# twice154/ofa-for-super-resolution

Measured on AMD Instinct MI355X. Metric: sr_training_images_per_sec_4x_64to256, higher is better.
Workload: dtype bf16; 1 GPU; OFA-SR S4 supernet 4x progressive shrinking (elastic kernel {3,5,7}, e=6, d=4, pd=2), LR 64x64 -> HR 256x256, fwd+bwd+Adam, train-mode BN; kernel_transform_mode=1, compat_reference_indexing=True, parallelism=dp1, per_gpu_batch=16, global_batch=16, grad_allreduce_bytes=0, launch=eager

## Files before the change

### ofa-for-super-resolution_amd/csrc/conv2d.hip

```cpp
#include "ofasr_common.h"

namespace ofasr {

typedef __attribute__((ext_vector_type(16))) float cv_f32x16;
typedef __attribute__((ext_vector_type(8))) __bf16 cv_bf16x8;
typedef __attribute__((ext_vector_type(8))) _Float16 cv_f16x8;
typedef __attribute__((ext_vector_type(8))) short cv_s16x8;

constexpr int CV_TW = 64;
constexpr int CV_SEG = 20;
constexpr int CV_RP = 4 * CV_SEG;
constexpr int CV_KC = 32;

template <typename T> struct CvMma;
template <> struct CvMma<bf16_t> {
    static __device__ __forceinline__ cv_f32x16 run(cv_s16x8 a, cv_s16x8 b, cv_f32x16 c) {
        return __builtin_amdgcn_mfma_f32_32x32x16_bf16(__builtin_bit_cast(cv_bf16x8, a), __builtin_bit_cast(cv_bf16x8, b),
                                                       c, 0, 0, 0);
    }
};
template <> struct CvMma<f16_t> {
    static __device__ __forceinline__ cv_f32x16 run(cv_s16x8 a, cv_s16x8 b, cv_f32x16 c) {
        return __builtin_amdgcn_mfma_f32_32x32x16_f16(__builtin_bit_cast(cv_f16x8, a), __builtin_bit_cast(cv_f16x8, b), c,
                                                      0, 0, 0);
    }
};

__device__ __forceinline__ int cv_pos(int r, int col) { return r * CV_RP + (col & 3) * CV_SEG + (col >> 2); }
__device__ __forceinline__ int cv_rec(int P, int j) { return P * 64 + ((j ^ ((P >> 2) & 3)) << 4); }

struct CvBn {
    float* ss;
    const float* gamma;
    const float* beta;
    const float* mean;
    const float* var;
    float eps;
};

template <typename T>
__global__ void __launch_bounds__(256) conv_prep_kernel(const float* __restrict__ w, T* __restrict__ wimg, int Cin,
                                                        int KS, int dgrad, int M, int Kdim, int nrb, long long total,
                                                        CvBn bn) {
    const long long idx = (long long)blockIdx.x * blockDim.x + threadIdx.x;
    if (bn.ss != nullptr && idx < M) {
        float sc = 1.f, sh = 0.f;
        if (bn.gamma != nullptr) {
            sc = bn.gamma[idx] * rsqrtf(bn.var[idx] + bn.eps);
            sh = bn.beta[idx] - bn.mean[idx] * sc;
        }
        bn.ss[idx] = sc;
        bn.ss[M + idx] = sh;
    }
    if (idx >= total) return;
    const int j = (int)(idx & 7), lane = (int)((idx >> 3) & 63);
    long long t = idx >> 9;
    const int rb = (int)(t % nrb);
    t /= nrb;
    const int tx = (int)(t % KS);
    t /= KS;
    const int s = (int)(t & 1);
    t >>= 1;
    const int ty = (int)(t % KS);
    const int kc = (int)(t / KS);
    const int m = rb * 32 + (lane & 31), kk = kc * CV_KC + 16 * s + 8 * (lane >> 5) + j;
    float v = 0.f;
    if (m < M && kk < Kdim) {
        const int taps = KS * KS, tap = ty * KS + tx;
        v = dgrad ? w[((long long)kk * Cin + m) * taps + (taps - 1 - tap)]
                  : w[((long long)m * Cin + kk) * taps + tap];
    }
    wimg[idx] = from_float<T>(v);
}

__device__ __forceinline__ void cv_lds_barrier() { asm volatile("s_waitcnt lgkmcnt(0)\n\ts_barrier" ::: "memory"); }

struct CvEpi {
    const float* ss;
    int act;
    float2* stat;
    int P;
};

template <typename T, int KS, int RB, int WM, int WP, bool ONEK>
__global__ void __launch_bounds__(64 * WM * WP, 2) conv_igemm_kernel(const T* __restrict__ x, const T* __restrict__ wimg,
                                                                     T* __restrict__ y, int Cx, int M, int H, int W,
                                                                     int tiles_x, int nkc, int nrb, CvEpi epi) {
    constexpr int THREADS = 64 * WM * WP;
    constexpr int PAD = KS / 2;
    constexpr int TH = 2 * WP;
    constexpr int RH = TH + KS - 1;
    constexpr int RW = CV_TW + KS - 1;
    constexpr int NIT = 2 * KS;
    __shared__ __attribute__((aligned(16))) char Xt[RH * CV_RP * 64];

    const int tile = blockIdx.x;
    const int ty0 = (tile / tiles_x) * TH, tx0 = (tile % tiles_x) * CV_TW;
    const int n = blockIdx.y, slab = blockIdx.z;
    const int tid = threadIdx.x;
    const int lane = lane_id();
    const int wave = __builtin_amdgcn_readfirstlane((int)(threadIdx.x >> 6));
    const int wm = wave % WM, wp = wave / WM;
    const int c = lane & 31, h = lane >> 5;
    const int prow = 2 * wp + (c >> 4), pcol = 4 * (c & 15);
    const int grb0 = (slab * WM + wm) * RB;

    const int P0 = prow * CV_RP + (c & 15);
    int bbase[2][4][2];
#pragma unroll
    for (int cs = 0; cs < 2; ++cs)
#pragma unroll
        for (int m = 0; m < 4; ++m)
#pragma unroll
            for (int ks = 0; ks < 2; ++ks) {
                const int key = (((P0 >> 2) & 3) + m + (cs && (c & 3) == 3 ? 1 : 0)) & 3;
                bbase[cs][m][ks] = P0 * 64 + (((2 * ks + h) ^ key) << 4);
            }
    auto read_b = [&](int ty, int u, int ks) -> cv_s16x8 {
        const int D = ty * CV_RP + (u & 3) * CV_SEG + (u >> 2);
        return *reinterpret_cast<const cv_s16x8*>(Xt + bbase[u >> 2][(D >> 2) & 3][ks] + D * 64);
    };

    cv_f32x16 acc[RB][4];
#pragma unroll
    for (int rb = 0; rb < RB; ++rb)
#pragma unroll
        for (int t = 0; t < 4; ++t)
#pragma unroll
            for (int i = 0; i < 16; ++i) acc[rb][t][i] = 0.f;

    const T* xn = x + (long long)n * Cx * H * W;
    const uint4* wbase = reinterpret_cast<const uint4*>(wimg);
    for (int kc = 0; kc < nkc; ++kc) {
        cv_s16x8 A[KS][RB];
        const long long it_stride = (long long)KS * nrb * 64;
        const uint4* wk = wbase + (long long)kc * NIT * it_stride + (long long)grb0 * 64;
#pragma unroll
        for (int tx = 0; tx < KS; ++tx)
#pragma unroll
            for (int rb = 0; rb < RB; ++rb)
                A[tx][rb] = __builtin_bit_cast(cv_s16x8, (wk + ((long long)tx * nrb + rb) * 64)[lane]);

        cv_lds_barrier();
        constexpr int NRUN = (CV_TW + 16) / 8;
        constexpr int NTASK = 4 * RH * NRUN;
#pragma unroll 1
        for (int q = tid; q < NTASK; q += THREADS) {
            const int run = q % NRUN;
            const int r = (q / NRUN) % RH;
            const int g = q / (NRUN * RH);
            const int gy = ty0 - PAD + r;
            const int gx = tx0 - 8 + 8 * run;
            const bool inb = gy >= 0 && gy < H && gx >= 0 && gx < W;
            const int cbase = CV_KC * kc + 8 * g;
            uint4 v[8];
#pragma unroll
            for (int i = 0; i < 8; ++i) {
                v[i] = make_uint4(0, 0, 0, 0);
                if (inb && cbase + i < Cx)
                    v[i] = *reinterpret_cast<const uint4*>(xn + ((long long)(cbase + i) * H + gy) * W + gx);
            }
#pragma unroll
            for (int k = 0; k < 4; ++k) {
                uint32_t lo[4], hi[4];
#pragma unroll
                for (int m = 0; m < 4; ++m) {
                    const uint32_t a = k == 0 ? v[2 * m].x : k == 1 ? v[2 * m].y : k == 2 ? v[2 * m].z : v[2 * m].w;
                    const uint32_t b = k == 0 ? v[2 * m + 1].x : k == 1 ? v[2 * m + 1].y : k == 2 ? v[2 * m + 1].z
                                                                                                  : v[2 * m + 1].w;
                    lo[m] = __builtin_amdgcn_perm(b, a, 0x05040100u);
                    hi[m] = __builtin_amdgcn_perm(b, a, 0x07060302u);
                }
                const int tc0 = 8 * run - 8 + PAD + 2 * k;
                if (tc0 >= 0 && tc0 < RW)
                    *reinterpret_cast<uint4*>(Xt + cv_rec(cv_pos(r, tc0), g)) = make_uint4(lo[0], lo[1], lo[2], lo[3]);
                if (tc0 + 1 >= 0 && tc0 + 1 < RW)
                    *reinterpret_cast<uint4*>(Xt + cv_rec(cv_pos(r, tc0 + 1), g)) = make_uint4(hi[0], hi[1], hi[2], hi[3]);
            }
        }
        cv_lds_barrier();

        constexpr int STEP = ONEK ? 2 : 1;
#pragma unroll
        for (int it = 0; it < NIT; it += STEP) {
            const int ty = it >> 1, ks = it & 1;
            cv_s16x8 B[8];
#pragma unroll
            for (int u = 0; u < KS + 3; ++u) B[u] = read_b(ty, u, ks);
#pragma unroll
            for (int tx = 0; tx < KS; ++tx) {
#pragma unroll
                for (int rb = 0; rb < RB; ++rb)
#pragma unroll
                    for (int t = 0; t < 4; ++t) acc[rb][t] = CvMma<T>::run(A[tx][rb], B[t + tx], acc[rb][t]);
                __builtin_amdgcn_sched_barrier(0);
                if (it + STEP < NIT) {
#pragma unroll
                    for (int rb = 0; rb < RB; ++rb)
                        A[tx][rb] = __builtin_bit_cast(
                            cv_s16x8, (wk + (it + STEP) * it_stride + ((long long)tx * nrb + rb) * 64)[lane]);
                }
                __builtin_amdgcn_sched_barrier(0);
            }
        }
    }
    const int oy = ty0 + prow, ox = tx0 + pcol;
    if (epi.ss != nullptr) {
        if (oy >= H || ox >= W) return;
#pragma unroll
        for (int rb = 0; rb < RB; ++rb) {
            const int mb = (grb0 + rb) * 32 + 4 * h;
#pragma unroll
            for (int q = 0; q < 4; ++q) {
                float v[4][4];
#pragma unroll
                for (int j = 0; j < 4; ++j) {
                    const int m = mb + 8 * q + j;
                    const int mc = m < M ? m : M - 1;
                    const float sc = epi.ss[mc], sh = epi.ss[M + mc];
#pragma unroll
                    for (int t = 0; t < 4; ++t) {
                        float r = fmaf(acc[rb][t][4 * q + j], sc, sh);
                        if (epi.act == 1) r = fminf(fmaxf(r, 0.f), 6.f);
                        v[j][t] = r;
                    }
                }
                if (epi.act == 2) {
                    const int m0 = mb + 8 * q;
                    if (m0 < M) {
                        T* dst = y + (((long long)n * (M >> 2) + (m0 >> 2)) * (2 * H) + 2 * oy) * (2 * W) + 2 * ox;
#pragma unroll
                        for (int dy = 0; dy < 2; ++dy)
                            *reinterpret_cast<uint4*>(dst + (long long)dy * (2 * W)) =
                                make_uint4(pack2<T>(v[2 * dy][0], v[2 * dy + 1][0]), pack2<T>(v[2 * dy][1], v[2 * dy + 1][1]),
                                           pack2<T>(v[2 * dy][2], v[2 * dy + 1][2]), pack2<T>(v[2 * dy][3], v[2 * dy + 1][3]));
                    }
                } else {
#pragma unroll
                    for (int j = 0; j < 4; ++j) {
                        const int m = mb + 8 * q + j;
                        if (m < M)
                            *reinterpret_cast<uint2*>(y + (((long long)n * M + m) * H + oy) * W + ox) =
                                make_uint2(pack2<T>(v[j][0], v[j][1]), pack2<T>(v[j][2], v[j][3]));
                    }
                }
            }
        }
        return;
    }
    const bool inside = oy < H && ox < W;
    if (inside) {
#pragma unroll
        for (int rb = 0; rb < RB; ++rb) {
#pragma unroll
            for (int reg = 0; reg < 16; ++reg) {
                const int m = (grb0 + rb) * 32 + (reg & 3) + 8 * (reg >> 2) + 4 * h;
                if (m < M) {
                    T* dst = y + (((long long)n * M + m) * H + oy) * W + ox;
                    *reinterpret_cast<uint2*>(dst) = make_uint2(pack2<T>(acc[rb][0][reg], acc[rb][1][reg]),
                                                                pack2<T>(acc[rb][2][reg], acc[rb][3][reg]));
                }
            }
        }
    }
    if (epi.stat != nullptr) {
        const int unit = (n * (int)gridDim.x + tile) * WP + wp;
#pragma unroll
        for (int rb = 0; rb < RB; ++rb) {
            float sv[16], qv[16];
#pragma unroll
            for (int reg = 0; reg < 16; ++reg) {
                float ss = 0.f, qq = 0.f;
#pragma unroll
                for (int t = 0; t < 4; ++t) {
                    const float v = inside ? to_float(from_float<T>(acc[rb][t][reg])) : 0.f;
                    ss += v;
                    qq = fmaf(v, v, qq);
                }
                sv[reg] = ss;
                qv[reg] = qq;
            }
            half_wave_row_sums(sv, qv, c);
            const int rho = half_wave_row_reg(c);
            const int m = (grb0 + rb) * 32 + (rho & 3) + 8 * (rho >> 2) + 4 * h;
            if ((c & 1) == 0 && m < M) epi.stat[(long long)m * epi.P + unit] = make_float2(sv[0], qv[0]);
        }
    }
}

struct CvPlan {
    bool ok;
    int cfg;
    int rows, th, threads, nslab, nrb, nkc, M, Kdim;
    size_t img_bytes;
};

static CvPlan cv_plan(int64_t Cin, int64_t Cout, int K, int dgrad, int64_t N = 0, int64_t H = 0, int64_t W = 0) {
    CvPlan p{};
    p.M = (int)(dgrad ? Cin : Cout);
    p.Kdim = (int)(dgrad ? Cout : Cin);
    p.ok = (K == 3 || K == 5) && p.M > 0 && p.Kdim > 0;
    p.cfg = p.M > 128 ? 0 : (p.M > 64 ? 1 : (p.M > 32 ? 2 : 3));
    if (p.cfg == 2 && N > 0 && N * cdiv(H, 8) * cdiv(W, CV_TW) < 512) p.cfg = 4;
    p.rows = p.cfg == 0 ? 256 : (p.cfg == 1 ? 128 : (p.cfg == 3 ? 32 : 64));
    p.th = p.cfg == 0 ? 2 : ((p.cfg == 1 || p.cfg == 4) ? 4 : 8);
    p.threads = 256;
    p.nslab = (int)cdiv(p.M, p.rows);
    p.nrb = p.nslab * (p.rows / 32);
    p.nkc = (int)cdiv(p.Kdim, CV_KC);
    p.img_bytes = (size_t)p.nkc * K * 2 * K * p.nrb * 1024;
    return p;
}

template <typename T>
static int launch_conv_prep(const char* name, const float* w, int64_t Cin, int64_t Cout, int K, int dgrad, void* ws, CvBn bn,
                            hipStream_t st) {
    const CvPlan p = cv_plan(Cin, Cout, K, dgrad);
    const long long total = (long long)(p.img_bytes / 2);
    OFASR_LAUNCH((conv_prep_kernel<T>), dim3((unsigned)cdiv(total, 256)), dim3(256), 0, st, w, (T*)ws, (int)Cin, K,
                       dgrad, p.M, p.Kdim, p.nrb, total, bn);
    return check_launch(name);
}

template <typename T>
static int launch_conv_run(const char* name, const void* x, const void* ws, void* y, int64_t N, int64_t Cin, int64_t Cout,
                           int64_t H, int64_t W, int K, int dgrad, CvEpi epi, hipStream_t st) {
    const CvPlan p = cv_plan(Cin, Cout, K, dgrad, N, H, W);
    const int tiles_x = (int)cdiv(W, CV_TW), tiles_y = (int)cdiv(H, p.th);
    dim3 grid((unsigned)(tiles_x * tiles_y), (unsigned)N, (unsigned)p.nslab);
    prof_note((double)sizeof(T) * (double)N * (double)H * (double)W * (double)(Cin + Cout),
              2.0 * (double)N * (double)H * (double)W * (double)Cin * (double)Cout * K * K);
#define OFASR_CV(KS, RB, WM, WP, ONEK)                                                                                  \
    OFASR_LAUNCH((conv_igemm_kernel<T, KS, RB, WM, WP, ONEK>), grid, dim3(64 * WM * WP), 0, st, (const T*)x,         \
                       (const T*)ws, (T*)y, p.Kdim, p.M, (int)H, (int)W, tiles_x, p.nkc, p.nrb, epi)
#define OFASR_CVK(KS, ONEK)                                                                                         \
    switch (p.cfg) {                                                                                                \
        case 0: OFASR_CV(KS, 2, 4, 1, ONEK); break;                                                                 \
        case 1: OFASR_CV(KS, 2, 2, 2, ONEK); break;                                                                 \
        case 2: OFASR_CV(KS, 2, 1, 4, ONEK); break;                                                                 \
        case 4: OFASR_CV(KS, 1, 2, 2, ONEK); break;                                                                 \
        default: OFASR_CV(KS, 1, 1, 4, ONEK); break;                                                                \
    }
    const bool onek = p.Kdim <= 16;
    if (K == 5) {
        if (onek) { OFASR_CVK(5, true) } else { OFASR_CVK(5, false) }
    } else {
        if (onek) { OFASR_CVK(3, true) } else { OFASR_CVK(3, false) }
    }
#undef OFASR_CVK
#undef OFASR_CV
    return check_launch(name);
}

template <typename T>
static int launch_conv2d(const char* name, const void* x, const float* w, void* y, int64_t N, int64_t Cin, int64_t Cout,
                         int64_t H, int64_t W, int K, int dgrad, void* ws, hipStream_t st, StatOut so = StatOut{nullptr, 0}) {
    int rc = launch_conv_prep<T>(name, w, Cin, Cout, K, dgrad, ws, CvBn{}, st);
    if (rc) return rc;
    return launch_conv_run<T>(name, x, ws, y, N, Cin, Cout, H, W, K, dgrad, CvEpi{nullptr, 0, so.partial, so.P}, st);
}

typedef __attribute__((ext_vector_type(4))) short cv_s16x4;
typedef __attribute__((address_space(3))) cv_s16x4 cv_lds_s16x4;

struct CvWgParams {
    int Cin, Cout, H, W, tiles_x, tiles_y, ntiles, ksplit, ncislab, nz;
};

template <int WCI> __device__ __forceinline__ int cvw_xoff(int R, int chunk) {
    if constexpr (WCI == 2) return R * 128 + ((((chunk >> 2) ^ ((R >> 1) & 1))) << 6) + ((chunk & 3) << 4);
    else return R * 64 + (chunk << 4);
}

template <typename T, int KS, int RBW, int WCO, int WCI, int WK>
__global__ void __launch_bounds__(256, 2) conv_wgrad_kernel(const T* __restrict__ dy, const T* __restrict__ x,
                                                            float* __restrict__ part, CvWgParams P) {
    static_assert(WCO * WCI * WK == 4, "4 waves");
    constexpr int PAD = KS / 2;
    constexpr int CIB = 32 * WCI;
    constexpr int REC = 2 * CIB;
    constexpr int ROWS = 32 * RBW * WCO;
    constexpr int XW = 80;
    __shared__ __attribute__((aligned(16))) char Yt[ROWS * 256];
    __shared__ __attribute__((aligned(16))) char Xt[2 * XW * REC];

    const int G = KS * P.nz;
    const int xcd = blockIdx.x & 7, jb = blockIdx.x >> 3;
    const int group = jb % G, split = (jb / G) * 8 + xcd;
    if (split >= P.ksplit) return;
    const int ty = group % KS, z = group / KS;
    const int coslab = z / P.ncislab, cislab = z % P.ncislab;
    const int tid = threadIdx.x, lane = lane_id();
    const int wave = __builtin_amdgcn_readfirstlane((int)(threadIdx.x >> 6));
    const int wco = wave % WCO, wci = (wave / WCO) % WCI, wk = wave / (WCO * WCI);
    const int c = lane & 31, h = lane >> 5;
    const int g = lane >> 4, q = (lane >> 2) & 3, pp = lane & 3;

    int xbase[2][2];
    {
        const int L = 8 * (g >> 1) + q;
        const int cb = 64 * wci + 32 * (g & 1) + 8 * pp;
#pragma unroll
        for (int b1 = 0; b1 < 2; ++b1)
#pragma unroll
            for (int b0 = 0; b0 < 2; ++b0) {
                if constexpr (WCI == 2) {
                    const int bit1 = ((L >> 1) & 1) ^ b1 ^ (b0 & L & 1);
                    xbase[b1][b0] = L * 128 + ((wci ^ bit1) << 6) + (cb & 63);
                } else {
                    xbase[b1][b0] = L * 64 + cb;
                }
            }
    }
    cv_f32x16 acc[RBW][KS];
#pragma unroll
    for (int rb = 0; rb < RBW; ++rb)
#pragma unroll
        for (int tx = 0; tx < KS; ++tx)
#pragma unroll
            for (int i = 0; i < 16; ++i) acc[rb][tx][i] = 0.f;

    const long long HW = (long long)P.H * P.W;
    const int t0 = (int)((long long)split * P.ntiles / P.ksplit), t1 = (int)((long long)(split + 1) * P.ntiles / P.ksplit);
    const int tpi = P.tiles_x * P.tiles_y;
    for (int tile = t0; tile < t1; ++tile) {
        const int n = tile / tpi, trem = tile - n * tpi;
        const int ty0 = (trem / P.tiles_x) * 2, tx0 = (trem % P.tiles_x) * CV_TW;
        const T* xn = x + (long long)n * P.Cin * HW;
        const T* dyn = dy + (long long)n * P.Cout * HW;
        __syncthreads();
        constexpr int NXT = (CIB / 8) * 2 * 10;
        if (tid < NXT) {
            const int run = tid % 10, r = (tid / 10) & 1, cg = tid / 20;
            const int gy = ty0 + r + ty - PAD, gx = tx0 - 8 + 8 * run;
            const bool inb = gy >= 0 && gy < P.H && gx >= 0 && gx < P.W;
            const int cbase = cislab * CIB + 8 * cg;
            uint4 v[8];
            uint32_t okm[8];
#pragma unroll
            for (int i = 0; i < 8; ++i) {
                const bool ok = inb && cbase + i < P.Cin;
                okm[i] = ok ? 0xffffffffu : 0u;
                v[i] = *reinterpret_cast<const uint4*>(xn + (ok ? ((long long)(cbase + i) * P.H + gy) * P.W + gx : 0));
            }
#pragma unroll
            for (int i = 0; i < 8; ++i) {
                v[i].x &= okm[i]; v[i].y &= okm[i]; v[i].z &= okm[i]; v[i].w &= okm[i];
            }
#pragma unroll
            for (int k = 0; k < 4; ++k) {
                uint32_t lo[4], hi[4];
#pragma unroll
                for (int m = 0; m < 4; ++m) {
                    const uint32_t a = k == 0 ? v[2 * m].x : k == 1 ? v[2 * m].y : k == 2 ? v[2 * m].z : v[2 * m].w;
                    const uint32_t b = k == 0 ? v[2 * m + 1].x : k == 1 ? v[2 * m + 1].y : k == 2 ? v[2 * m + 1].z
                                                                                                  : v[2 * m + 1].w;
                    lo[m] = __builtin_amdgcn_perm(b, a, 0x05040100u);
                    hi[m] = __builtin_amdgcn_perm(b, a, 0x07060302u);
                }
                const int R = r * XW + 8 * run + 2 * k;
                *reinterpret_cast<uint4*>(Xt + cvw_xoff<WCI>(R, cg)) = make_uint4(lo[0], lo[1], lo[2], lo[3]);
                *reinterpret_cast<uint4*>(Xt + cvw_xoff<WCI>(R + 1, cg)) = make_uint4(hi[0], hi[1], hi[2], hi[3]);
            }
        }
        constexpr int NYT = ROWS * 16;
#pragma unroll
        for (int i0 = 0; i0 < NYT; i0 += 4 * 256) {
            uint4 v[4];
            uint32_t okm[4];
#pragma unroll
            for (int j = 0; j < 4; ++j) {
                const int idx = i0 + j * 256 + tid;
                const int chunk = idx & 15, row = idx >> 4;
                const int co = coslab * ROWS + row, gy = ty0 + (chunk >> 3), gx = tx0 + 8 * (chunk & 7);
                const bool ok = idx < NYT && co < P.Cout && gy < P.H && gx < P.W;
                okm[j] = ok ? 0xffffffffu : 0u;
                v[j] = *reinterpret_cast<const uint4*>(dyn + (ok ? ((long long)co * P.H + gy) * P.W + gx : 0));
            }
#pragma unroll
            for (int j = 0; j < 4; ++j) {
                const int idx = i0 + j * 256 + tid;
                const int chunk = idx & 15, row = idx >> 4;
                v[j].x &= okm[j]; v[j].y &= okm[j]; v[j].z &= okm[j]; v[j].w &= okm[j];
                if (idx < NYT) *reinterpret_cast<uint4*>(Yt + row * 256 + ((chunk ^ (row & 15)) << 4)) = v[j];
            }
        }
        __syncthreads();
#pragma unroll
        for (int s = 0; s < 8; ++s) {
            if ((s % WK) != wk) continue;
            cv_s16x8 A[RBW];
#pragma unroll
            for (int rb = 0; rb < RBW; ++rb) {
                const int row = 32 * (wco * RBW + rb) + c;
                A[rb] = *reinterpret_cast<const cv_s16x8*>(Yt + row * 256 + (((2 * s + h) ^ (row & 15)) << 4));
            }
#pragma unroll
            for (int tx = 0; tx < KS; ++tx) {
                const int Da = (s >> 2) * XW + 16 * (s & 3) + 8 - PAD + tx, Db = Da + 4;
                const cv_s16x4 lo = __builtin_amdgcn_ds_read_tr16_b64_v4i16(
                    (cv_lds_s16x4*)(Xt + xbase[(Da >> 1) & 1][Da & 1] + Da * REC));
                const cv_s16x4 hi = __builtin_amdgcn_ds_read_tr16_b64_v4i16(
                    (cv_lds_s16x4*)(Xt + xbase[(Db >> 1) & 1][Db & 1] + Db * REC));
                const cv_s16x8 B = __builtin_shufflevector(lo, hi, 0, 1, 2, 3, 4, 5, 6, 7);
#pragma unroll
                for (int rb = 0; rb < RBW; ++rb) acc[rb][tx] = CvMma<T>::run(A[rb], B, acc[rb][tx]);
            }
        }
    }
    const int wq = wave % (WCO * WCI);
    if constexpr (WK > 1) {
        static_assert(WCO * WCI * RBW * 4096 <= ROWS * 256, "Yt holds one tx slice per (wco, wci)");
        float* red = reinterpret_cast<float*>(Yt) + wq * (RBW * 16 * 64) + lane;
#pragma unroll
        for (int tx = 0; tx < KS; ++tx) {
#pragma unroll
            for (int ph = 1; ph < WK; ++ph) {
                __syncthreads();
                if (wk == ph) {
#pragma unroll
                    for (int rb = 0; rb < RBW; ++rb)
#pragma unroll
                        for (int reg = 0; reg < 16; ++reg) red[(rb * 16 + reg) * 64] = acc[rb][tx][reg];
                }
                __syncthreads();
                if (wk == 0) {
#pragma unroll
                    for (int rb = 0; rb < RBW; ++rb)
#pragma unroll
                        for (int reg = 0; reg < 16; ++reg) acc[rb][tx][reg] += red[(rb * 16 + reg) * 64];
                }
            }
        }
        if (wk != 0) return;
    }
    float* dst = part + ((((long long)split * KS + ty) * P.nz + z) * (WCO * WCI) + wq) * (RBW * KS * 16 * 64) + lane;
#pragma unroll
    for (int rb = 0; rb < RBW; ++rb)
#pragma unroll
        for (int tx = 0; tx < KS; ++tx)
#pragma unroll
            for (int reg = 0; reg < 16; ++reg) dst[((rb * KS + tx) * 16 + reg) * 64] = acc[rb][tx][reg];
}

template <int KS, int RBW, int WCO, int WCI>
__global__ void __launch_bounds__(256) conv_wgrad_reduce_kernel(const float* __restrict__ part, float* __restrict__ dw,
                                                                CvWgParams P, long long total) {
    const long long idx = (long long)blockIdx.x * blockDim.x + threadIdx.x;
    if (idx >= total) return;
    constexpr int PER_WAVE = RBW * KS * 16 * 64;
    long long t = idx;
    const int lane = (int)(t & 63);
    t >>= 6;
    const int reg = (int)(t & 15);
    t >>= 4;
    const int tx = (int)(t % KS);
    t /= KS;
    const int rb = (int)(t % RBW);
    t /= RBW;
    const int wq = (int)(t % (WCO * WCI));
    t /= (WCO * WCI);
    const int z = (int)(t % P.nz);
    const int ty = (int)(t / P.nz);
    const int wco = wq % WCO, wci = wq / WCO;
    const int coslab = z / P.ncislab, cislab = z % P.ncislab;
    const int co = coslab * (32 * RBW * WCO) + 32 * (wco * RBW + rb) + (reg & 3) + 8 * (reg >> 2) + 4 * (lane >> 5);
    const int ci = cislab * (32 * WCI) + 32 * wci + (lane & 31);
    if (co >= P.Cout || ci >= P.Cin) return;
    const long long inner = ((long long)(rb * KS + tx) * 16 + reg) * 64 + lane;
    float sum = 0.f;
    const long long sstride = (long long)KS * P.nz * (WCO * WCI) * PER_WAVE;
    const float* src = part + (((long long)ty * P.nz + z) * (WCO * WCI) + wq) * PER_WAVE + inner;
    for (int split = 0; split < P.ksplit; ++split) sum += src[split * sstride];
    dw[(((long long)co * P.Cin + ci) * KS + ty) * KS + tx] = sum;
}

struct CvWgPlan {
    int cfg;
    int rows, cib, rbw;
    CvWgParams P;
    size_t part_bytes;
    double note_bytes, note_flops;
};

static CvWgPlan cv_wg_plan(int64_t N, int64_t Cin, int64_t Cout, int64_t H, int64_t W, int K) {
    CvWgPlan p{};
    p.note_bytes = 2.0 * (double)N * (double)H * (double)W * (double)(Cin + Cout);
    p.note_flops = 2.0 * (double)N * (double)H * (double)W * (double)Cin * (double)Cout * K * K;
    const bool wide = Cin > 32;
    const int rcls = Cout > 64 ? 0 : (Cout > 32 ? 1 : 2);
    p.cfg = (wide ? 0 : 3) + rcls;
    p.rows = rcls == 0 ? 128 : (rcls == 1 ? 64 : 32);
    p.rbw = rcls == 2 ? 1 : 2;
    p.cib = wide ? 64 : 32;
    CvWgParams& P = p.P;
    P.Cin = (int)Cin; P.Cout = (int)Cout; P.H = (int)H; P.W = (int)W;
    P.tiles_x = (int)cdiv(W, CV_TW); P.tiles_y = (int)cdiv(H, 2);
    P.ntiles = (int)(N * P.tiles_x * P.tiles_y);
    P.ncislab = (int)cdiv(Cin, p.cib);
    P.nz = (int)cdiv(Cout, p.rows) * P.ncislab;
    int ks = 512 / (K * P.nz);
    ks = ks > P.ntiles / 8 ? P.ntiles / 8 : ks;
    if (ks > 8) ks -= ks % 8;
    P.ksplit = ks < 1 ? 1 : ks;
    const int nwq = wide ? (rcls == 0 ? 4 : 2) : (rcls == 0 ? 2 : 1);
    p.part_bytes = (size_t)P.ksplit * K * P.nz * nwq * (p.rbw * K * 16 * 64) * sizeof(float);
    return p;
}

template <typename T>
static int launch_conv2d_wgrad(const char* name, const void* dy, const void* x, float* dw, int K, const CvWgPlan& p, void* ws,
                               hipStream_t st) {
    const CvWgParams& P = p.P;
    dim3 grid((unsigned)(cdiv(P.ksplit, 8) * 8 * K * P.nz));
    prof_note(p.note_bytes, p.note_flops);
#define OFASR_WG(KS, RBW, WCO, WCI, WK)                                                                              \
    {                                                                                                                \
        OFASR_LAUNCH((conv_wgrad_kernel<T, KS, RBW, WCO, WCI, WK>), grid, dim3(256), 0, st, (const T*)dy,      \
                           (const T*)x, (float*)ws, P);                                                              \
        int rc = check_launch(name);                                                                                 \
        if (rc) return rc;                                                                                           \
        const long long tot = (long long)KS * P.nz * (WCO * WCI) * RBW * KS * 16 * 64;                               \
        OFASR_LAUNCH((conv_wgrad_reduce_kernel<KS, RBW, WCO, WCI>), dim3((unsigned)cdiv(tot, 256)),            \
                           dim3(256), 0, st, (const float*)ws, dw, P, tot);                                          \
    }
#define OFASR_WGK(KS)                                                                                                \
    switch (p.cfg) {                                                                                                 \
        case 0: OFASR_WG(KS, 2, 2, 2, 1) break;                                                                      \
        case 1: OFASR_WG(KS, 2, 1, 2, 2) break;                                                                      \
        case 2: OFASR_WG(KS, 1, 1, 2, 2) break;                                                                      \
        case 3: OFASR_WG(KS, 2, 2, 1, 2) break;                                                                      \
        case 4: OFASR_WG(KS, 2, 1, 1, 4) break;                                                                      \
        default: OFASR_WG(KS, 1, 1, 1, 4) break;                                                                     \
    }
    if (K == 5) { OFASR_WGK(5) } else { OFASR_WGK(3) }
#undef OFASR_WGK
#undef OFASR_WG
    return check_launch(name);
}

static int conv_stat_units(int64_t N, int64_t Cin, int64_t Cout, int64_t H, int64_t W, int K) {
    if (conv_thin_out_supported(Cout, Cin, K, W, OFASR_BF16, nullptr, nullptr))
        return conv_thin_out_units(N, Cout, Cin, H, W, OFASR_BF16);
    if (conv_thin_in_supported(Cin, Cout, K, W, OFASR_BF16, nullptr, nullptr))
        return conv_thin_in_units(N, Cin, Cout, H, W, OFASR_BF16);
    const CvPlan p = cv_plan(Cin, Cout, K, 0, N, H, W);
    const int wp = p.th / 2;
    return (int)(N * cdiv(W, CV_TW) * cdiv(H, p.th) * wp);
}

static int conv2d_entry(const char* name, const void* x, const float* w, void* y, int64_t N, int64_t Cin, int64_t Cout,
                        int64_t H, int64_t W, int K, int dtype, int dgrad, void* ws, size_t ws_bytes, void* stream,
                        StatOut so = StatOut{nullptr, 0}) {
    OFASR_REQUIRE(x && w && y, OFASR_ERR_INVALID_ARG, "%s: null pointer", name);
    OFASR_REQUIRE(N > 0 && Cin > 0 && Cout > 0 && H > 0 && W > 0, OFASR_ERR_INVALID_ARG, "%s: bad shape", name);
    OFASR_REQUIRE(dtype == OFASR_F16 || dtype == OFASR_BF16, OFASR_ERR_UNSUPPORTED,
                  "%s: 16-bit activations only (fp32 runs on the vendor library)", name);
    OFASR_REQUIRE(K == 3 || K == 5, OFASR_ERR_UNSUPPORTED, "%s: K=%d not in {3,5}", name, K);
    OFASR_REQUIRE(W % 8 == 0 && ((reinterpret_cast<uintptr_t>(x) | reinterpret_cast<uintptr_t>(y)) & 15) == 0,
                  OFASR_ERR_UNSUPPORTED, "%s: needs W %% 8 == 0 and 16-byte aligned tensors", name);
    OFASR_REQUIRE(N <= 65535 && H * W <= (1LL << 31), OFASR_ERR_UNSUPPORTED, "%s: too large", name);
    const CvPlan p = cv_plan(Cin, Cout, K, dgrad);
    OFASR_REQUIRE(ws && ws_bytes >= p.img_bytes, OFASR_ERR_WORKSPACE, "%s: workspace %zu B < required %zu B", name,
                  ws_bytes, p.img_bytes);
    hipStream_t st = as_stream(stream);
    {
        const int64_t Ct = dgrad ? Cin : Cout, Cw = dgrad ? Cout : Cin;
        if (conv_thin_out_supported(Ct, Cw, K, W, dtype, x, y)) {
            if (so.partial)
                OFASR_REQUIRE(!dgrad && so.P == conv_thin_out_units(N, Ct, Cw, H, W, dtype), OFASR_ERR_INVALID_ARG,
                              "%s: statistics unit count %d does not match the launch", name, so.P);
            return conv_thin_out(x, w, y, N, Ct, Cw, H, W, K, dtype, dgrad, so, stream);
        }
        if (conv_thin_in_supported(Cw, Ct, K, W, dtype, x, y)) {
            if (so.partial)
                OFASR_REQUIRE(!dgrad && so.P == conv_thin_in_units(N, Cw, Ct, H, W, dtype), OFASR_ERR_INVALID_ARG,
                              "%s: statistics unit count %d does not match the launch", name, so.P);
            return conv_thin_in(x, w, y, N, Cw, Ct, H, W, K, dtype, dgrad, so, stream);
        }
    }
    if (so.partial)
        OFASR_REQUIRE(!dgrad && so.P == conv_stat_units(N, Cin, Cout, H, W, K), OFASR_ERR_INVALID_ARG,
                      "%s: statistics unit count %d does not match the launch", name, so.P);
    if (dtype == OFASR_BF16) return launch_conv2d<bf16_t>(name, x, w, y, N, Cin, Cout, H, W, K, dgrad, ws, st, so);
    return launch_conv2d<f16_t>(name, x, w, y, N, Cin, Cout, H, W, K, dgrad, ws, st, so);
}

}

using namespace ofasr;

OFASR_EXPORT size_t ofasr_conv2d_workspace(int64_t Cin, int64_t Cout, int K, int dgrad) {
    if (Cin <= 0 || Cout <= 0 || !(K == 3 || K == 5)) return 0;
    return cv_plan(Cin, Cout, K, dgrad).img_bytes;
}

OFASR_EXPORT int ofasr_conv2d_fwd(const void* x, const float* w, void* y, int64_t N, int64_t Cin, int64_t Cout, int64_t H,
                                  int64_t W, int K, int dtype, void* workspace, size_t workspace_bytes, void* stream) {
    return conv2d_entry("ofasr_conv2d_fwd", x, w, y, N, Cin, Cout, H, W, K, dtype, 0, workspace, workspace_bytes, stream);
}

static size_t cv_infer_bytes(int64_t Cin, int64_t Cout, int K) {
    return (cv_plan(Cin, Cout, K, 0).img_bytes + 255) / 256 * 256 + (size_t)(2 * Cout) * sizeof(float);
}
OFASR_EXPORT size_t ofasr_conv2d_infer_operand_bytes(int64_t Cin, int64_t Cout, int K) {
    if (Cin <= 0 || Cout <= 0 || !(K == 3 || K == 5)) return 0;
    return cv_infer_bytes(Cin, Cout, K);
}

OFASR_EXPORT int ofasr_conv2d_infer_prepare(const float* w, const float* gamma, const float* beta, const float* running_mean,
                                            const float* running_var, double eps, int64_t Cin, int64_t Cout, int K, int dtype,
                                            void* operands, size_t operand_bytes, void* stream) {
    const char* name = "ofasr_conv2d_infer_prepare";
    OFASR_REQUIRE(w && operands, OFASR_ERR_INVALID_ARG, "%s: null pointer", name);
    OFASR_REQUIRE(Cin > 0 && Cout > 0, OFASR_ERR_INVALID_ARG, "%s: bad shape", name);
    OFASR_REQUIRE(dtype == OFASR_F16 || dtype == OFASR_BF16, OFASR_ERR_UNSUPPORTED, "%s: 16-bit activations only", name);
    OFASR_REQUIRE(K == 3 || K == 5, OFASR_ERR_UNSUPPORTED, "%s: K=%d not in {3,5}", name, K);
    OFASR_REQUIRE(gamma == nullptr || (beta && running_mean && running_var), OFASR_ERR_INVALID_ARG, "%s: incomplete BN", name);
    OFASR_REQUIRE(operand_bytes >= cv_infer_bytes(Cin, Cout, K), OFASR_ERR_WORKSPACE, "%s: operand buffer %zu B < required %zu B",
                  name, operand_bytes, cv_infer_bytes(Cin, Cout, K));
    float* ss = reinterpret_cast<float*>((char*)operands + (cv_plan(Cin, Cout, K, 0).img_bytes + 255) / 256 * 256);
    const CvBn bn{ss, gamma, beta, running_mean, running_var, (float)eps};
    hipStream_t st = as_stream(stream);
    if (dtype == OFASR_BF16) return launch_conv_prep<bf16_t>(name, w, Cin, Cout, K, 0, operands, bn, st);
    return launch_conv_prep<f16_t>(name, w, Cin, Cout, K, 0, operands, bn, st);
}

OFASR_EXPORT int ofasr_conv2d_infer_run(const void* x, void* y, int64_t N, int64_t Cin, int64_t Cout, int64_t H, int64_t W,
                                        int K, int dtype, int act, const void* operands, size_t operand_bytes, void* stream) {
    const char* name = "ofasr_conv2d_infer_run";
    OFASR_REQUIRE(x && y && operands, OFASR_ERR_INVALID_ARG, "%s: null pointer", name);
    OFASR_REQUIRE(N > 0 && Cin > 0 && Cout > 0 && H > 0 && W > 0, OFASR_ERR_INVALID_ARG, "%s: bad shape", name);
    OFASR_REQUIRE(dtype == OFASR_F16 || dtype == OFASR_BF16, OFASR_ERR_UNSUPPORTED, "%s: 16-bit activations only", name);
    OFASR_REQUIRE(K == 3 || K == 5, OFASR_ERR_UNSUPPORTED, "%s: K=%d not in {3,5}", name, K);
    OFASR_REQUIRE(act >= 0 && act <= 2, OFASR_ERR_INVALID_ARG, "%s: act %d not in {0 none, 1 relu6, 2 pixel shuffle}", name, act);
    OFASR_REQUIRE(act != 2 || Cout % 4 == 0, OFASR_ERR_INVALID_ARG, "%s: PixelShuffle(2) needs Cout %% 4 == 0", name);
    OFASR_REQUIRE(W % 8 == 0 && ((reinterpret_cast<uintptr_t>(x) | reinterpret_cast<uintptr_t>(y)) & 15) == 0,
                  OFASR_ERR_UNSUPPORTED, "%s: needs W %% 8 == 0 and 16-byte aligned tensors", name);
    OFASR_REQUIRE(N <= 65535 && H * W <= (1LL << 29), OFASR_ERR_UNSUPPORTED, "%s: too large", name);
    OFASR_REQUIRE(operand_bytes >= cv_infer_bytes(Cin, Cout, K), OFASR_ERR_WORKSPACE, "%s: operand buffer %zu B < required %zu B",
                  name, operand_bytes, cv_infer_bytes(Cin, Cout, K));
    const float* ss = reinterpret_cast<const float*>((const char*)operands + (cv_plan(Cin, Cout, K, 0).img_bytes + 255) / 256 * 256);
    hipStream_t st = as_stream(stream);
    if (dtype == OFASR_BF16) return launch_conv_run<bf16_t>(name, x, operands, y, N, Cin, Cout, H, W, K, 0, CvEpi{ss, act, nullptr, 0}, st);
    return launch_conv_run<f16_t>(name, x, operands, y, N, Cin, Cout, H, W, K, 0, CvEpi{ss, act, nullptr, 0}, st);
}

OFASR_EXPORT int ofasr_conv2d_stat_units(int64_t N, int64_t Cin, int64_t Cout, int64_t H, int64_t W, int K) {
    if (N <= 0 || Cin <= 0 || Cout <= 0 || H <= 0 || W <= 0 || !(K == 3 || K == 5)) return 0;
    return conv_stat_units(N, Cin, Cout, H, W, K);
}

OFASR_EXPORT int ofasr_conv2d_fwd_stat(const void* x, const float* w, void* y, int64_t N, int64_t Cin, int64_t Cout, int64_t H,
                                       int64_t W, int K, int dtype, void* partial, int64_t units, void* workspace,
                                       size_t workspace_bytes, void* stream) {
    OFASR_REQUIRE(partial != nullptr && units > 0 && units <= INT32_MAX, OFASR_ERR_INVALID_ARG,
                  "ofasr_conv2d_fwd_stat: null / empty statistics buffer");
    return conv2d_entry("ofasr_conv2d_fwd_stat", x, w, y, N, Cin, Cout, H, W, K, dtype, 0, workspace, workspace_bytes, stream,
                        StatOut{(float2*)partial, (int)units});
}

OFASR_EXPORT int ofasr_conv2d_dgrad(const void* dy, const float* w, void* dx, int64_t N, int64_t Cin, int64_t Cout,
                                    int64_t H, int64_t W, int K, int dtype, void* workspace, size_t workspace_bytes,
                                    void* stream) {
    return conv2d_entry("ofasr_conv2d_dgrad", dy, w, dx, N, Cin, Cout, H, W, K, dtype, 1, workspace, workspace_bytes,
                        stream);
}

OFASR_EXPORT size_t ofasr_conv2d_wgrad_workspace(int64_t N, int64_t Cin, int64_t Cout, int64_t H, int64_t W, int K) {
    if (N <= 0 || Cin <= 0 || Cout <= 0 || H <= 0 || W <= 0 || !(K == 3 || K == 5)) return 0;
    size_t need = cv_wg_plan(N, Cin, Cout, H, W, K).part_bytes;
    const int64_t Ct = Cin < Cout ? Cin : Cout, Cw = Cin < Cout ? Cout : Cin;
    if (conv_thin_wgrad_supported(Ct, Cw, K, H, W, OFASR_BF16, nullptr, nullptr)) {
        const size_t thin = conv_thin_wgrad_workspace(N, Ct, Cw, H, W, K, OFASR_BF16);
        need = thin > need ? thin : need;
    }
    return need;
}

OFASR_EXPORT int ofasr_conv2d_wgrad(const void* dy, const void* x, float* dw, int64_t N, int64_t Cin, int64_t Cout,
                                    int64_t H, int64_t W, int K, int dtype, void* workspace, size_t workspace_bytes,
                                    void* stream) {
    const char* name = "ofasr_conv2d_wgrad";
    OFASR_REQUIRE(dy && x && dw, OFASR_ERR_INVALID_ARG, "%s: null pointer", name);
    OFASR_REQUIRE(N > 0 && Cin > 0 && Cout > 0 && H > 0 && W > 0, OFASR_ERR_INVALID_ARG, "%s: bad shape", name);
    OFASR_REQUIRE(dtype == OFASR_F16 || dtype == OFASR_BF16, OFASR_ERR_UNSUPPORTED,
                  "%s: 16-bit activations only (fp32 runs on the vendor library)", name);
    OFASR_REQUIRE(K == 3 || K == 5, OFASR_ERR_UNSUPPORTED, "%s: K=%d not in {3,5}", name, K);
    OFASR_REQUIRE(W % 8 == 0 && ((reinterpret_cast<uintptr_t>(x) | reinterpret_cast<uintptr_t>(dy)) & 15) == 0,
                  OFASR_ERR_UNSUPPORTED, "%s: needs W %% 8 == 0 and 16-byte aligned tensors", name);
    OFASR_REQUIRE(N * H * W <= (1LL << 30), OFASR_ERR_UNSUPPORTED, "%s: too large", name);
    {
        const int64_t Ct = Cin < Cout ? Cin : Cout, Cw = Cin < Cout ? Cout : Cin;
        if (conv_thin_wgrad_supported(Ct, Cw, K, H, W, dtype, dy, x))
            return conv_thin_wgrad(dy, x, dw, N, Cin, Cout, H, W, K, dtype, workspace, workspace_bytes, stream);
    }
    const CvWgPlan p = cv_wg_plan(N, Cin, Cout, H, W, K);
    OFASR_REQUIRE(workspace && workspace_bytes >= p.part_bytes, OFASR_ERR_WORKSPACE,
                  "%s: workspace %zu B < required %zu B", name, workspace_bytes, p.part_bytes);
    hipStream_t st = as_stream(stream);
    if (dtype == OFASR_BF16) return launch_conv2d_wgrad<bf16_t>(name, dy, x, dw, K, p, workspace, st);
    return launch_conv2d_wgrad<f16_t>(name, dy, x, dw, K, p, workspace, st);
}
```

Baseline: 2721 images/s.

## Add warp-specialized double-buffered loader kernel for wide conv weight gradients

Adds a 512-thread weight-gradient kernel in which four producer waves prefetch dY and X tiles from global memory into registers and deposit them into double-buffered LDS. Four consumer waves run MFMA on the other buffer. For the widest config, each block also processes two k-splits and writes one partial slab per split, which halves the grid. The aim is to overlap global loads with MFMA compute in the wgrad pass. The cost is a larger dynamic LDS footprint and lower occupancy. The path is on by default for wide shapes and can be turned off with an environment variable.

```diff
diff --git a/ofa-for-super-resolution_amd/csrc/conv2d.hip b/ofa-for-super-resolution_amd/csrc/conv2d.hip
--- a/ofa-for-super-resolution_amd/csrc/conv2d.hip
+++ b/ofa-for-super-resolution_amd/csrc/conv2d.hip
@@ -365,6 +365,7 @@
 
 struct CvWgParams {
     int Cin, Cout, H, W, tiles_x, tiles_y, ntiles, ksplit, ncislab, nz;
+    int spb;
 };
 
 template <int WCI> __device__ __forceinline__ int cvw_xoff(int R, int chunk) {
@@ -541,6 +542,222 @@
         for (int tx = 0; tx < KS; ++tx)
 #pragma unroll
             for (int reg = 0; reg < 16; ++reg) dst[((rb * KS + tx) * 16 + reg) * 64] = acc[rb][tx][reg];
+}
+
+template <typename T, int KS, int RBW, int WCO, int WCI, int WK>
+__global__ void __launch_bounds__(512) conv_wgrad_kernel_ld(const T* __restrict__ dy, const T* __restrict__ x,
+                                                            float* __restrict__ part, CvWgParams P) {
+    static_assert(WCI == 2 && WCO * WCI * WK == 4, "4 compute waves on 64-channel slabs");
+    constexpr int PAD = KS / 2;
+    constexpr int CIB = 64, REC = 128;
+    constexpr int ROWS = 32 * RBW * WCO;
+    constexpr int XW = 80;
+    constexpr int YB = ROWS * 256, BUF = YB + 2 * XW * REC;
+    constexpr int NRED = WK > 1 ? 2 * KS * (WK - 1) : 0;
+    extern __shared__ __attribute__((aligned(16))) char cvl_smem[];
+
+    const int G = KS * P.nz;
+    const int xcd = blockIdx.x & 7, jb = blockIdx.x >> 3;
+    const int group = jb % G, split0 = ((jb / G) * 8 + xcd) * P.spb;
+    if (split0 >= P.ksplit) return;
+    const int split1 = split0 + P.spb < P.ksplit ? split0 + P.spb : P.ksplit;
+    const int ty = group % KS, z = group / KS;
+    const int coslab = z / P.ncislab, cislab = z % P.ncislab;
+    const int tid = threadIdx.x, lane = lane_id();
+    const int wave = __builtin_amdgcn_readfirstlane((int)(threadIdx.x >> 6));
+    const long long HW = (long long)P.H * P.W;
+    auto bound = [&](int sp) { return (int)((long long)sp * P.ntiles / P.ksplit); };
+    const int t0 = bound(split0), t1 = bound(split1);
+    const int nt = t1 - t0;
+    const int tpi = P.tiles_x * P.tiles_y;
+
+    if (wave >= 4) {
+        const int lt = tid - 256;
+        const int tl = lane < 40 ? lane : lane - 40;
+        const int cg = tl & 7, rr = (wave - 4) * 5 + (tl >> 3);
+        const int run = rr % 10, r = rr / 10;
+        const int chunk = lt & 15, rowl = lt >> 4;
+        constexpr int NJ = ROWS / 16;
+        unsigned xch[8], ych[NJ];
+        uint32_t xcm[8], ycm[NJ];
+#pragma unroll
+        for (int i = 0; i < 8; ++i) {
+            const int ch = cislab * CIB + 8 * cg + i;
+            xcm[i] = ch < P.Cin ? 0xffffffffu : 0u;
+            xch[i] = (unsigned)(ch < P.Cin ? ch : 0) * (unsigned)HW * 2u;
+        }
+#pragma unroll
+        for (int j = 0; j < NJ; ++j) {
+            const int co = coslab * ROWS + 16 * j + rowl;
+            ycm[j] = co < P.Cout ? 0xffffffffu : 0u;
+            ych[j] = (unsigned)(co < P.Cout ? co : 0) * (unsigned)HW * 2u;
+        }
+        const int ydst = rowl * 256 + ((chunk ^ rowl) << 4);
+        uint4 xv[8], yv[NJ];
+        uint32_t xm = 0u, ym = 0u;
+        auto request = [&](int tile) {
+            const int n = tile / tpi, trem = tile - n * tpi;
+            const int ty0 = (trem / P.tiles_x) * 2, tx0 = (trem % P.tiles_x) * CV_TW;
+            const char* xn = reinterpret_cast<const char*>(x + (long long)n * P.Cin * HW);
+            const char* dyn = reinterpret_cast<const char*>(dy + (long long)n * P.Cout * HW);
+            const int gy = ty0 + r + ty - PAD, gx = tx0 - 8 + 8 * run;
+            const bool inb = (gy >= 0) & (gy < P.H) & (gx >= 0) & (gx < P.W);
+            xm = inb ? 0xffffffffu : 0u;
+            const unsigned xo = inb ? (unsigned)(gy * P.W + gx) * 2u : 0u;
+#pragma unroll
+            for (int i = 0; i < 8; ++i) xv[i] = *reinterpret_cast<const uint4*>(xn + (xch[i] + xo));
+            const int yy = ty0 + (chunk >> 3), yx = tx0 + 8 * (chunk & 7);
+            const bool yin = (yy < P.H) & (yx < P.W);
+            ym = yin ? 0xffffffffu : 0u;
+            const unsigned yo = yin ? (unsigned)(yy * P.W + yx) * 2u : 0u;
+#pragma unroll
+            for (int j = 0; j < NJ; ++j) yv[j] = *reinterpret_cast<const uint4*>(dyn + (ych[j] + yo));
+        };
+        auto deposit = [&](char* Yt) {
+            char* Xt = Yt + YB;
+#pragma unroll
+            for (int i = 0; i < 8; ++i) {
+                const uint32_t m = xm & xcm[i];
+                xv[i].x &= m; xv[i].y &= m; xv[i].z &= m; xv[i].w &= m;
+            }
+#pragma unroll
+            for (int k = 0; k < 4; ++k) {
+                uint32_t lo[4], hi[4];
+#pragma unroll
+                for (int m = 0; m < 4; ++m) {
+                    const uint32_t a = k == 0 ? xv[2 * m].x : k == 1 ? xv[2 * m].y : k == 2 ? xv[2 * m].z : xv[2 * m].w;
+                    const uint32_t b = k == 0 ? xv[2 * m + 1].x : k == 1 ? xv[2 * m + 1].y : k == 2 ? xv[2 * m + 1].z
+                                                                                                    : xv[2 * m + 1].w;
+                    lo[m] = __builtin_amdgcn_perm(b, a, 0x05040100u);
+                    hi[m] = __builtin_amdgcn_perm(b, a, 0x07060302u);
+                }
+                const int R = r * XW + 8 * run + 2 * k;
+                *reinterpret_cast<uint4*>(Xt + cvw_xoff<2>(R, cg)) = make_uint4(lo[0], lo[1], lo[2], lo[3]);
+                *reinterpret_cast<uint4*>(Xt + cvw_xoff<2>(R + 1, cg)) = make_uint4(hi[0], hi[1], hi[2], hi[3]);
+            }
+#pragma unroll
+            for (int j = 0; j < NJ; ++j) {
+                const uint32_t m = ym & ycm[j];
+                yv[j].x &= m; yv[j].y &= m; yv[j].z &= m; yv[j].w &= m;
+                *reinterpret_cast<uint4*>(Yt + ydst + j * 4096) = yv[j];
+            }
+        };
+        if (nt > 0) {
+            request(t0);
+            deposit(cvl_smem);
+        }
+        if (nt > 1) request(t0 + 1);
+        cv_lds_barrier();
+        for (int i = 0; i < nt; ++i) {
+            if (i + 1 < nt) deposit(cvl_smem + ((i + 1) & 1) * BUF);
+            if (i + 2 < nt) request(t0 + i + 2);
+            cv_lds_barrier();
+        }
+#pragma unroll 1
+        for (int b = 0; b < NRED; ++b) cv_lds_barrier();
+        return;
+    }
+
+    const int wco = wave % WCO, wci = (wave / WCO) % WCI, wk = wave / (WCO * WCI);
+    const int c = lane & 31, h = lane >> 5;
+    const int g = lane >> 4, q = (lane >> 2) & 3, pp = lane & 3;
+    int xbase[2][2];
+    {
+        const int L = 8 * (g >> 1) + q;
+        const int cb = 64 * wci + 32 * (g & 1) + 8 * pp;
+#pragma unroll
+        for (int b1 = 0; b1 < 2; ++b1)
+#pragma unroll
+            for (int b0 = 0; b0 < 2; ++b0) {
+                const int bit1 = ((L >> 1) & 1) ^ b1 ^ (b0 & L & 1);
+                xbase[b1][b0] = L * 128 + ((wci ^ bit1) << 6) + (cb & 63);
+            }
+    }
+    cv_f32x16 acc[RBW][KS];
+#pragma unroll
+    for (int rb = 0; rb < RBW; ++rb)
+#pragma unroll
+        for (int tx = 0; tx < KS; ++tx)
+#pragma unroll
+            for (int i = 0; i < 16; ++i) acc[rb][tx][i] = 0.f;
+
+    const int wq = wave % (WCO * WCI);
+    auto store_slab = [&](int sp) {
+        float* dst = part + ((((long long)sp * KS + ty) * P.nz + z) * (WCO * WCI) + wq) * (RBW * KS * 16 * 64) + lane;
+#pragma unroll
+        for (int rb = 0; rb < RBW; ++rb)
+#pragma unroll
+            for (int tx = 0; tx < KS; ++tx)
+#pragma unroll
+                for (int reg = 0; reg < 16; ++reg) dst[((rb * KS + tx) * 16 + reg) * 64] = acc[rb][tx][reg];
+    };
+    int split = split0, tb = bound(split0 + 1) - t0;
+    cv_lds_barrier();
+    for (int i = 0; i < nt; ++i) {
+        const char* Yt = cvl_smem + (i & 1) * BUF;
+        const char* Xt = Yt + YB;
+#pragma unroll
+        for (int s = 0; s < 8; ++s) {
+            if ((s % WK) != wk) continue;
+            cv_s16x8 A[RBW];
+#pragma unroll
+            for (int rb = 0; rb < RBW; ++rb) {
+                const int row = 32 * (wco * RBW + rb) + c;
+                A[rb] = *reinterpret_cast<const cv_s16x8*>(Yt + row * 256 + (((2 * s + h) ^ (row & 15)) << 4));
+            }
+#pragma unroll
+            for (int tx = 0; tx < KS; ++tx) {
+                const int Da = (s >> 2) * XW + 16 * (s & 3) + 8 - PAD + tx, Db = Da + 4;
+                const cv_s16x4 lo = __builtin_amdgcn_ds_read_tr16_b64_v4i16(
+                    (cv_lds_s16x4*)(Xt + xbase[(Da >> 1) & 1][Da & 1] + Da * REC));
+                const cv_s16x4 hi = __builtin_amdgcn_ds_read_tr16_b64_v4i16(
+                    (cv_lds_s16x4*)(Xt + xbase[(Db >> 1) & 1][Db & 1] + Db * REC));
+                const cv_s16x8 B = __builtin_shufflevector(lo, hi, 0, 1, 2, 3, 4, 5, 6, 7);
+#pragma unroll
+                for (int rb = 0; rb < RBW; ++rb) acc[rb][tx] = CvMma<T>::run(A[rb], B, acc[rb][tx]);
+            }
+        }
+        cv_lds_barrier();
+        if constexpr (WK == 1) {
+            if (i + 1 == tb && i + 1 < nt) {
+                store_slab(split);
+#pragma unroll
+                for (int rb = 0; rb < RBW; ++rb)
+#pragma unroll
+                    for (int tx = 0; tx < KS; ++tx)
+#pragma unroll
+                        for (int r = 0; r < 16; ++r) acc[rb][tx][r] = 0.f;
+                ++split;
+                tb = bound(split + 1) - t0;
+            }
+        }
+    }
+    if constexpr (WK > 1) {
+        static_assert(WCO * WCI * RBW * 4096 <= ROWS * 256, "the dY image holds one tx slice per (wco, wci)");
+        float* red = reinterpret_cast<float*>(cvl_smem) + wq * (RBW * 16 * 64) + lane;
+#pragma unroll
+        for (int tx = 0; tx < KS; ++tx) {
+#pragma unroll
+            for (int ph = 1; ph < WK; ++ph) {
+                cv_lds_barrier();
+                if (wk == ph) {
+#pragma unroll
+                    for (int rb = 0; rb < RBW; ++rb)
+#pragma unroll
+                        for (int reg = 0; reg < 16; ++reg) red[(rb * 16 + reg) * 64] = acc[rb][tx][reg];
+                }
+                cv_lds_barrier();
+                if (wk == 0) {
+#pragma unroll
+                    for (int rb = 0; rb < RBW; ++rb)
+#pragma unroll
+                        for (int reg = 0; reg < 16; ++reg) acc[rb][tx][reg] += red[(rb * 16 + reg) * 64];
+                }
+            }
+        }
+        if (wk != 0) return;
+    }
+    store_slab(split);
 }
 
 template <int KS, int RBW, int WCO, int WCI>
@@ -578,10 +795,16 @@
 struct CvWgPlan {
     int cfg;
     int rows, cib, rbw;
+    bool loader;
     CvWgParams P;
     size_t part_bytes;
     double note_bytes, note_flops;
 };
+
+static bool cv_wg_loader_enabled() {
+    static const bool on = [] { const char* e = getenv("OFASR_CONV_WGRAD_LOADER"); return !(e && e[0] == '0'); }();
+    return on;
+}
 
 static CvWgPlan cv_wg_plan(int64_t N, int64_t Cin, int64_t Cout, int64_t H, int64_t W, int K) {
     CvWgPlan p{};
@@ -599,10 +822,12 @@
     P.ntiles = (int)(N * P.tiles_x * P.tiles_y);
     P.ncislab = (int)cdiv(Cin, p.cib);
     P.nz = (int)cdiv(Cout, p.rows) * P.ncislab;
+    p.loader = cv_wg_loader_enabled() && wide && rcls < 2 && (Cin > Cout ? Cin : Cout) * H * W < (1LL << 30);
     int ks = 512 / (K * P.nz);
     ks = ks > P.ntiles / 8 ? P.ntiles / 8 : ks;
     if (ks > 8) ks -= ks % 8;
     P.ksplit = ks < 1 ? 1 : ks;
+    P.spb = p.loader && p.cfg == 0 ? 2 : 1;
     const int nwq = wide ? (rcls == 0 ? 4 : 2) : (rcls == 0 ? 2 : 1);
     p.part_bytes = (size_t)P.ksplit * K * P.nz * nwq * (p.rbw * K * 16 * 64) * sizeof(float);
     return p;
@@ -612,7 +837,7 @@
 static int launch_conv2d_wgrad(const char* name, const void* dy, const void* x, float* dw, int K, const CvWgPlan& p, void* ws,
                                hipStream_t st) {
     const CvWgParams& P = p.P;
-    dim3 grid((unsigned)(cdiv(P.ksplit, 8) * 8 * K * P.nz));
+    dim3 grid((unsigned)(cdiv(cdiv(P.ksplit, P.spb), 8) * 8 * K * P.nz));
     prof_note(p.note_bytes, p.note_flops);
 #define OFASR_WG(KS, RBW, WCO, WCI, WK)                                                                              \
     {                                                                                                                \
@@ -624,7 +849,25 @@
         OFASR_LAUNCH((conv_wgrad_reduce_kernel<KS, RBW, WCO, WCI>), dim3((unsigned)cdiv(tot, 256)),            \
                            dim3(256), 0, st, (const float*)ws, dw, P, tot);                                          \
     }
+#define OFASR_WGL(KS, RBW, WCO, WCI, WK)                                                                             \
+    {                                                                                                                \
+        constexpr int lds = 2 * (32 * RBW * WCO * 256 + 2 * 80 * 128);                                               \
+        static const bool attr = ((void)hipFuncSetAttribute(                                                         \
+            reinterpret_cast<const void*>(&conv_wgrad_kernel_ld<T, KS, RBW, WCO, WCI, WK>),                          \
+            hipFuncAttributeMaxDynamicSharedMemorySize, lds), true);                                                 \
+        (void)attr;                                                                                                  \
+        OFASR_LAUNCH((conv_wgrad_kernel_ld<T, KS, RBW, WCO, WCI, WK>), grid, dim3(512), lds, st, (const T*)dy,       \
+                           (const T*)x, (float*)ws, P);                                                              \
+        int rc = check_launch(name);                                                                                 \
+        if (rc) return rc;                                                                                           \
+        const long long tot = (long long)KS * P.nz * (WCO * WCI) * RBW * KS * 16 * 64;                               \
+        OFASR_LAUNCH((conv_wgrad_reduce_kernel<KS, RBW, WCO, WCI>), dim3((unsigned)cdiv(tot, 256)),            \
+                           dim3(256), 0, st, (const float*)ws, dw, P, tot);                                          \
+    }
 #define OFASR_WGK(KS)                                                                                                \
+    if (p.loader) {                                                                                                  \
+        if (p.cfg == 0) OFASR_WGL(KS, 2, 2, 2, 1) else OFASR_WGL(KS, 2, 1, 2, 2)                                     \
+    } else                                                                                                           \
     switch (p.cfg) {                                                                                                 \
         case 0: OFASR_WG(KS, 2, 2, 2, 1) break;                                                                      \
         case 1: OFASR_WG(KS, 2, 1, 2, 2) break;                                                                      \
@@ -635,6 +878,7 @@
     }
     if (K == 5) { OFASR_WGK(5) } else { OFASR_WGK(3) }
 #undef OFASR_WGK
+#undef OFASR_WGL
 #undef OFASR_WG
     return check_launch(name);
 }
```

Result: no change. 2743 images/s (median of 6 runs) (+0.8%).
